# shenwei356/wfa

Measured on AMD Instinct MI355X. Metric: aligned pairs/sec (and Gcells/s) on 1e6 synthetic 1 kbp pairs @5% error, higher is better.
Workload: dtype u32; 1 GPU; 1000000 x 1000 bp pairs/GPU @5% error, global gap-affine 4/6/2, wf-adaptive 10/50/1, seed 3; config=c3, pairs_per_gpu=1000000, length=1000, parallelism=pair-sharded x1, ranks_seen_by_collective=1, backend=none (1 GPU), collective_forced=False, status_ok=1000000, setup_steps=0, gather=none (1 GPU), gather_bytes_per_rank_step=0, packed_pairs=1000000, retried_pairs=831

## Files before the change

wfa_amd/csrc/wfa_duo.hpp:

```cpp
#pragma once
#include "wfa_blk.hpp"
#include "wfa_duo_cfg.hpp"
#include "wfa_pk16.hpp"

namespace wfa {

struct DuoRed {
#define WFA_DUO_3(opa, opb, opc)                                                                                    \
    unsigned long long sv;                                                                                          \
    asm volatile("s_nop 1\n\t" opa " %0, %0, %0 " WFA_DPP_CTL_XOR1 "\n\t" opb " %1, %1, %1 " WFA_DPP_CTL_XOR1 "\n\t" opc \
        " %2, %2, %2 " WFA_DPP_CTL_XOR1 "\n\t" opa " %0, %0, %0 " WFA_DPP_CTL_XOR2 "\n\t" opb " %1, %1, %1 "        \
        WFA_DPP_CTL_XOR2 "\n\t" opc " %2, %2, %2 " WFA_DPP_CTL_XOR2 "\n\t" opa " %0, %0, %0 " WFA_DPP_CTL_HMIR "\n\t" \
        opb " %1, %1, %1 " WFA_DPP_CTL_HMIR "\n\t" opc " %2, %2, %2 " WFA_DPP_CTL_HMIR "\n\t"                         \
        "s_and_saveexec_b64 %3, %4\n\t" opa " %0, %0, %0 " WFA_DPP_CTL_MIR "\n\t" opb " %1, %1, %1 " WFA_DPP_CTL_MIR    \
        "\n\t" opc " %2, %2, %2 " WFA_DPP_CTL_MIR "\n\ts_mov_b64 exec, %3"                                            \
        : "+v"(a), "+v"(b), "+v"(c), "=&s"(sv)                                                                      \
        : "s"(wm)                                                                                                   \
        : "scc");
#define WFA_DUO_2(opa, opb)                                                                                         \
    unsigned long long sv;                                                                                          \
    asm volatile("s_nop 1\n\t" opa " %0, %0, %0 " WFA_DPP_CTL_XOR1 "\n\t" opb " %1, %1, %1 " WFA_DPP_CTL_XOR1 "\n\ts_nop 0\n\t" \
        opa " %0, %0, %0 " WFA_DPP_CTL_XOR2 "\n\t" opb " %1, %1, %1 " WFA_DPP_CTL_XOR2 "\n\ts_nop 0\n\t" opa        \
        " %0, %0, %0 " WFA_DPP_CTL_HMIR "\n\t" opb " %1, %1, %1 " WFA_DPP_CTL_HMIR "\n\t"                            \
        "s_and_saveexec_b64 %2, %3\n\t" opa " %0, %0, %0 " WFA_DPP_CTL_MIR "\n\t" opb " %1, %1, %1 " WFA_DPP_CTL_MIR    \
// ... 37 lines not shown

    const uint32_t  SW = P.lds_seq_words, PW = P.prepack_words;
    const uint32_t  FP = duo_fetch_pairs(PW), NBUF = duo_bufs(PW);
    uint32_t *const park0 = lds + NBUF * PW;
    const uint64_t  cap      = P.arena_words;
    const int       mdd      = (int)P.max_dist_diff;
    const int       minwf    = (int)P.min_wf_len;
    const bool      adaptive = P.adaptive != 0;
    const uint32_t  seed_si  = P.dx;
    uint32_t        pk_one   = 0x00010001u;
    if constexpr (PK) asm volatile("" : "+s"(pk_one));
    const int       rows_cap = (int)(cap / 32);

    int       st = 0;
    bool      wide = false;
    uint32_t  pidx = 0, si = 0, cells = 0, sbuf = 0;
    int       n = 0, m = 0, kb = 0;
    bool      slow = false, first_eq = false;
    int             j = l7, k0 = 0;
    uint32_t        mdn = 0u, mup = 0u;
    const uint32_t *lq = lds + 4, *lt = lds + 4;
    uint32_t       *rowp = nullptr;

    uint32_t M[R][RW], I[RW], D[RW];
    int      rlo[R], rhi[R];
    int      lim[PP], lmx[PP];
#pragma unroll
    for (int d = 0; d < R; d++) {
        rlo[d] = BK_BIG, rhi[d] = -BK_BIG;
#pragma unroll
        for (int p = 0; p < RW; p++) M[d][p] = 0u;
    }
#pragma unroll
    for (int p = 0; p < RW; p++) I[p] = D[p] = 0u;
#pragma unroll
    for (int p = 0; p < PP; p++) lim[p] = 0, lmx[p] = 0;

    uint32_t buf_free  = (1u << NBUF) - 1u;
    uint32_t park_used = 0u;
    constexpr uint32_t PF_TOK = 1u, PF_LD = 2u, PF_STAGED = 4u, PF_DRY = 8u;
    uint32_t pf = 0u;
    uint32_t pf_tok = 0u, pf_ld_idx = 0u, pf_idx = 0u, pf_buf = 0u;
    uint32_t st_mask = 0u;
    uint4    pf_w = make_uint4(0u, 0u, 0u, 0u);

#ifdef WFA_STAMPS
    unsigned long long stamp_acc[8] = {0, 0, 0, 0, 0, 0, 0, 0}, stamp_prev;
    unsigned long long evt[8] = {0, 0, 0, 0, 0, 0, 0, 0};
    asm volatile("s_memtime %0\n\ts_waitcnt lgkmcnt(0)" : "=s"(stamp_prev)::"memory");
#endif
    const auto pair_of = [&](uint32_t idx) { return P.work ? P.work[idx] : P.chunk_first + idx; };
    const auto dn1 = [&](uint32_t x) { return (uint32_t)__builtin_amdgcn_update_dpp(0, (int)x, 0x111, 0xf, 0xf, true) & mdn; };
    const auto up1 = [&](uint32_t x) { return (uint32_t)__builtin_amdgcn_update_dpp(0, (int)x, 0x101, 0xf, 0xf, true) & mup; };
    const auto other_half = [&](int x) { return __builtin_amdgcn_update_dpp(0, x, 0x128, 0xf, 0xf, true); };
    const auto set_derived = [&]() {
        j   = wide ? l15 : l7;
        mdn = j == 0 ? 0u : ~0u;
        mup = j == (wide ? 15 : 7) ? 0u : ~0u;
        k0  = kb + PP * j;
#pragma unroll
        for (int p = 0; p < PP; p++) lim[p] = imax2(1, imin2(n + k0 + p, m)), lmx[p] = imax2(n + k0 + p, m);
        lq   = lds + sbuf * PW + 4u;
        lt   = lq + SW;
        if constexpr (DUO_ARENA_FMT == 10u)
            rowp = P.arena + (uint64_t)pidx * cap + (((uint32_t)k0 & 56u) >> 3) * (uint32_t)(rows_cap * 4) + (((uint32_t)k0 >> 2) & 1u) * 16u;
        else if constexpr (DUO_ARENA_FMT == 9u)
            rowp = P.arena + (uint64_t)pidx * cap + (((uint32_t)k0 & 60u) >> 2) * (uint32_t)(rows_cap * 2) + si * 2u;
        else
            rowp = P.arena + (uint64_t)pidx * cap + (uint64_t)(si >> 3) * 256u + (si & 7u) * 2u;
    };
    const auto clear_rings = [&]() {
#pragma unroll
        for (int d = 0; d < R; d++) {
            rlo[d] = BK_BIG, rhi[d] = -BK_BIG;
#pragma unroll
            for (int p = 0; p < RW; p++) M[d][p] = 0u;
        }
#pragma unroll
        for (int p = 0; p < RW; p++) I[p] = D[p] = 0u;
    };
    const auto or_halves = [&](uint32_t v) {
        uint32_t r = 0u;
#pragma unroll
        for (int o = 0; o < 8; o++) r |= (uint32_t)__builtin_amdgcn_readlane((int)v, 8 * o);
        return r;
    };

    const auto refill = [&](auto ph_c) __attribute__((always_inline)) -> bool {
        constexpr int ph  = decltype(ph_c)::value;
        constexpr int NEW = (ph + R - 1) % R;
        pf        = (uint32_t)__builtin_amdgcn_readfirstlane((int)pf);
        park_used = (uint32_t)__builtin_amdgcn_readfirstlane((int)park_used);
        buf_free  = (uint32_t)__builtin_amdgcn_readfirstlane((int)buf_free);
        st_mask   = (uint32_t)__builtin_amdgcn_readfirstlane((int)st_mask);
        if ((pf & (PF_LD | PF_STAGED)) == PF_LD) {
            const uint32_t cnt = umin2(FP, P.chunk_n - pf_ld_idx);
            st_mask = 0u;
            {
                uint32_t f = buf_free;
                for (uint32_t c = 0; c < cnt; c++) st_mask |= f & (0u - f), f &= f - 1u;
            }
            buf_free &= ~st_mask;
            const uint32_t w0 = (uint32_t)lane * 4u, slot = w0 / PW;
            if (slot < cnt) {
                uint32_t f = st_mask;
                for (uint32_t c = 0; c < slot; c++) f &= f - 1u;
                const uint32_t b = (uint32_t)__builtin_ctz(f);
                *reinterpret_cast<uint4 *>(lds + b * PW + (w0 - slot * PW)) = pf_w;
            }
            pf_idx = pf_ld_idx, pf = (pf | PF_STAGED) & ~PF_LD;
        }
        if ((pf & (PF_TOK | PF_LD)) == PF_TOK) {
            pf_ld_idx = (uint32_t)__builtin_amdgcn_readfirstlane((int)pf_tok);
            const bool have = pf_ld_idx < P.chunk_n;
            if (have) {
                const uint32_t *const slot = P.prepack + (uint64_t)pf_ld_idx * PW;
                const uint32_t cnt = umin2(FP, P.chunk_n - pf_ld_idx);
                if ((uint32_t)lane * 4u < cnt * PW) pf_w = *reinterpret_cast<const uint4 *>(slot + lane * 4);
            }
            pf = (pf & ~PF_TOK) | (have ? PF_LD : PF_DRY);
        }
        if ((pf & (PF_TOK | PF_DRY)) == 0u) {
            if (lane == 0) pf_tok = atomicAdd(P.queue_head, FP);
            pf |= PF_TOK;
        }
        unsigned long long m_free;
        WFA_STAMP(0);
        for (;;) {
        const bool run   = st == 1;
        const int  Wc    = wide ? 64 : 32;
        const bool touch = run && rhi[NEW] >= rlo[NEW] && (rlo[NEW] <= kb || rhi[NEW] >= kb + Wc - 1);
        bool       narrowable = false;
        if constexpr (ph == 0) {
            int ulo = rlo[0], uhi = rhi[0];
#pragma unroll
            for (int d = 1; d < R; d++) ulo = imin2(ulo, rlo[d]), uhi = imax2(uhi, rhi[d]);
            narrowable    = run && wide && uhi - ulo + 1 <= DUO_NARROW_AT;
        }
        const unsigned long long m_ev = __ballot(touch || narrowable);
        m_free = __ballot(st == 0);
        if (__builtin_expect(!(m_ev != 0ull || (m_free != 0ull && (park_used != 0u || (pf & PF_STAGED) != 0u))), 1)) break;
        WFA_EVT(1, 1);
        {
            int ulo = rlo[0], uhi = rhi[0];
#pragma unroll
            for (int d = 1; d < R; d++) ulo = imin2(ulo, rlo[d]), uhi = imax2(uhi, rhi[d]);
            const int span = uhi - ulo + 1;
            int act = 0;
            if (touch) act = wide ? (span > DUO_WIDE_MAX ? 4 : 1) : (span > DUO_WIDEN_AT ? 2 : 1);
            else if (narrowable) act = 3;
            const int Wn  = act == 2 ? 64 : (act == 3 ? 32 : Wc);
            const int kbn = (((ulo + uhi + 1 - Wn) >> 1) + 2) & ~3;
            if (act != 0 && act != 4 && !(ulo - kbn >= 1 && uhi - kbn <= Wn - 2)) act = 4;
            const int  o_act = other_half(act), o_kb = other_half(kb), o_kbn = other_half(kbn);
            const bool o_wide = other_half(wide ? 1 : 0) != 0;
            bool widen  = act == 2 && !(hi_half && o_act == 2);
            bool taken  = !wide && !o_wide && o_act == 2 && !(!hi_half && act == 2);
            bool evict  = taken && st == 1;
            unsigned long long m_evict = __ballot(evict);
            bool               lost    = false;
            while (m_evict != 0ull) {
                const int      l0   = __builtin_ctzll(m_evict);
                const uint32_t oct  = (uint32_t)l0 >> 3;
                m_evict &= ~(0xFFull << (8 * oct));
                const bool mine = evict && ((uint32_t)lane >> 3) == oct;
                if (park_used == (1u << DUO_PARK) - 1u) {
                    if (((uint32_t)lane >> 3) == (oct ^ 1u)) lost = true;
                    if (mine) evict = false, taken = false;
                    continue;
                }
                const uint32_t rec = (uint32_t)__builtin_ctz(~park_used);
                park_used |= 1u << rec;
                WFA_EVT(3, 1);
                uint32_t *const pr = park0 + rec * DUO_PARK_WORDS;
                if (mine) {
                    uint4 *const w = reinterpret_cast<uint4 *>(pr + 12 * l7);
                    const auto pk  = [](uint32_t lo, uint32_t hi) { return lo | (hi << 16); };
                    const auto pk2 = [&](const uint32_t(&v)[RW], int h) -> uint32_t {
                        if constexpr (PK) return v[h];
                        else return pk(v[2 * h], v[2 * h + 1]);
                    };
                    uint32_t pw[8];
                    int      plo[4], phi[4];
#pragma unroll
                    for (int r = 0; r < 4; r++) {
                        pw[2 * r]     = r < R ? pk2(M[(ph + r) % R], 0) : 0u;
                        pw[2 * r + 1] = r < R ? pk2(M[(ph + r) % R], 1) : 0u;
                        plo[r] = r < R ? rlo[(ph + r) % R] : BK_BIG, phi[r] = r < R ? rhi[(ph + r) % R] : -BK_BIG;
                    }
                    w[0] = make_uint4(pw[0], pw[1], pw[2], pw[3]);
                    if constexpr (R > 2) w[1] = make_uint4(pw[4], pw[5], pw[6], pw[7]);
                    w[2] = make_uint4(pk2(I, 0), pk2(I, 1), pk2(D, 0), pk2(D, 1));
                    if (l7 == 0) {
                        uint4 *const s4 = reinterpret_cast<uint4 *>(pr + 96);
                        s4[0] = make_uint4(pidx, si, cells, sbuf);
                        s4[1] = make_uint4((uint32_t)n, (uint32_t)m, (uint32_t)kb, (slow ? 1u : 0u) | (first_eq ? 2u : 0u));
                        s4[2] = make_uint4((uint32_t)plo[0], (uint32_t)plo[1], (uint32_t)plo[2], (uint32_t)plo[3]);
                        s4[3] = make_uint4((uint32_t)phi[0], (uint32_t)phi[1], (uint32_t)phi[2], (uint32_t)phi[3]);
                    }
                }
            }
            if (lost) widen = false, act = 4;
            {
                const bool o_lost = other_half(lost ? 1 : 0) != 0;
                if (o_lost) taken = false;
            }
            if (__ballot(act == 4) != 0ull) {
                WFA_EVT(7, __builtin_popcountll(__ballot(act == 4 && j == 0)));
                if (act == 4 && j == 0) {
                    P.pair_meta[pidx] = make_uint4(ST_REDO_BAND, 0u, 0u, 0u);
                    push_redo(P, pair_of(pidx), ST_REDO_BAND);
                }
                buf_free |= or_halves(act == 4 ? (1u << sbuf) : 0u);
                if (act == 4) {
                    st = 0, wide = false;
                    clear_rings();
                }
            }
            const int  rb   = lane & ~15;
            const bool join = taken;
            int src = lane;
            bool moved = false, freed = false;
            {
                if (join) {
                    const int Bo = (lane & ~7) ^ 8, dl = (o_kbn - o_kb) >> 2, jo = (lane - rb) + dl;
                    src = (jo >= 0 && jo < 8) ? Bo + jo : -1, moved = true;
                } else if (act == 1) {
                    const int Bo = wide ? rb : (lane & ~7), Go = wide ? 16 : 8, dl = (kbn - kb) >> 2, jo = (lane - Bo) + dl;
// ... 13 lines not shown
                const int sl = (src < 0 ? lane : src) << 2;
#pragma unroll
                for (int d = 0; d < R; d++)
#pragma unroll
                    for (int p = 0; p < RW; p++) {
                        const uint32_t v = (uint32_t)__builtin_amdgcn_ds_bpermute(sl, (int)M[d][p]);
                        M[d][p]          = src < 0 ? 0u : v;
                    }
#pragma unroll
                for (int p = 0; p < RW; p++) {
                    const uint32_t v = (uint32_t)__builtin_amdgcn_ds_bpermute(sl, (int)I[p]);
                    const uint32_t u = (uint32_t)__builtin_amdgcn_ds_bpermute(sl, (int)D[p]);
                    I[p] = src < 0 ? 0u : v, D[p] = src < 0 ? 0u : u;
                }
                if (__ballot(join) != 0ull) {
                    const int      o_n = other_half(n), o_m = other_half(m);
                    const uint32_t o_pidx = (uint32_t)other_half((int)pidx), o_si = (uint32_t)other_half((int)si);
                    const uint32_t o_cells = (uint32_t)other_half((int)cells), o_sbuf = (uint32_t)other_half((int)sbuf);
                    const int      o_fl = other_half((slow ? 1 : 0) | (first_eq ? 2 : 0));
                    int o_rlo[R], o_rhi[R];
#pragma unroll
                    for (int d = 0; d < R; d++) o_rlo[d] = other_half(rlo[d]), o_rhi[d] = other_half(rhi[d]);
                    if (join) {
                        n = o_n, m = o_m, pidx = o_pidx, si = o_si, cells = o_cells, sbuf = o_sbuf;
                        slow = (o_fl & 1) != 0, first_eq = (o_fl & 2) != 0;
#pragma unroll
                        for (int d = 0; d < R; d++) rlo[d] = o_rlo[d], rhi[d] = o_rhi[d];
                        st = 1;
                    }
                }
                if (join) kb = o_kbn;
                else if (moved && !freed) kb = kbn;
                if (join || widen) wide = true;
                if (act == 3) wide = false;
                if (freed) {
                    st = 0;
#pragma unroll
                    for (int d = 0; d < R; d++) rlo[d] = BK_BIG, rhi[d] = -BK_BIG;
                }
            }
            m_free = __ballot(st == 0);
            while (m_free != 0ull && (park_used != 0u || (pf & PF_STAGED) != 0u)) {
                const uint32_t oct  = (uint32_t)__builtin_ctzll(m_free) >> 3;
                const bool     mine = ((uint32_t)lane >> 3) == oct;
                if (park_used != 0u) {
                    const uint32_t rec = (uint32_t)__builtin_ctz(park_used);
                    park_used &= park_used - 1u;
                    WFA_EVT(4, 1);
                    const uint32_t *const pr = park0 + rec * DUO_PARK_WORDS;
                    if (mine) {
                        const uint4 *const w = reinterpret_cast<const uint4 *>(pr + 12 * l7);
                        const uint4 v0 = w[0], v1 = R > 2 ? w[1] : make_uint4(0u, 0u, 0u, 0u), v2 = w[2];
                        const uint32_t pw[8] = {v0.x, v0.y, v0.z, v0.w, v1.x, v1.y, v1.z, v1.w};
                        const uint4 *const s4 = reinterpret_cast<const uint4 *>(pr + 96);
                        const uint4 a0 = s4[0], a1 = s4[1], a2 = s4[2], a3 = s4[3];
                        const uint32_t plo[4] = {a2.x, a2.y, a2.z, a2.w}, phi[4] = {a3.x, a3.y, a3.z, a3.w};
#pragma unroll
                        for (int r = 0; r < R; r++) {
                            if constexpr (PK) {
                                M[(ph + r) % R][0] = pw[2 * r], M[(ph + r) % R][1] = pw[2 * r + 1];
                            } else {
                                M[(ph + r) % R][0] = pw[2 * r] & 0xFFFFu, M[(ph + r) % R][1] = pw[2 * r] >> 16;
                                M[(ph + r) % R][2] = pw[2 * r + 1] & 0xFFFFu, M[(ph + r) % R][3] = pw[2 * r + 1] >> 16;
                            }
                            rlo[(ph + r) % R] = (int)plo[r], rhi[(ph + r) % R] = (int)phi[r];
                        }
                        if constexpr (PK) {
                            I[0] = v2.x, I[1] = v2.y, D[0] = v2.z, D[1] = v2.w;
                        } else {
                            I[0] = v2.x & 0xFFFFu, I[1] = v2.x >> 16, I[2] = v2.y & 0xFFFFu, I[3] = v2.y >> 16;
                            D[0] = v2.z & 0xFFFFu, D[1] = v2.z >> 16, D[2] = v2.w & 0xFFFFu, D[3] = v2.w >> 16;
                        }
                        pidx = a0.x, si = a0.y, cells = a0.z, sbuf = a0.w;
                        n = (int)a1.x, m = (int)a1.y, kb = (int)a1.z, slow = (a1.w & 1u) != 0u, first_eq = (a1.w & 2u) != 0u;
                        st = 1, wide = false;
                    }
                    m_free &= ~(0xFFull << (8 * oct));
                    continue;
                }
                pf_buf   = (uint32_t)__builtin_ctz(st_mask);
                st_mask &= st_mask - 1u;
                const uint32_t this_idx = pf_idx;
                pf_idx += 1u;
                const uint32_t *const hb = lds + pf_buf * PW;
                const uint32_t nq = (uint32_t)__builtin_amdgcn_readfirstlane((int)hb[0]), mt = (uint32_t)__builtin_amdgcn_readfirstlane((int)hb[1]);
                const uint32_t status = (uint32_t)__builtin_amdgcn_readfirstlane((int)hb[2]);
                if (st_mask == 0u) pf &= ~PF_STAGED;
                if (status != ST_PENDING) {
                    if (lane == 0) {
                        P.pair_meta[this_idx] = make_uint4(status, 0u, 0u, 0u);
                        if (status >= ST_REDO_BYTES) push_redo(P, pair_of(this_idx), status);
                    }
                    buf_free |= 1u << pf_buf;
                    continue;
                }
                WFA_EVT(5, 1);
                if (mine) {
                    pidx = this_idx, sbuf = pf_buf;
                    n = (int)nq, m = (int)mt;
                    const int Ak = m - n;
                    si = 0, cells = 0, slow = false;
                    kb = -16 + PP * imax2(-3, imin2(3, Ak / (2 * PP)));
                    first_eq = ((hb[4] ^ hb[4 + SW]) & 3u) == 0u;
                    clear_rings();
                    st = 1, wide = false;
                }
                m_free &= ~(0xFFull << (8 * oct));
            }
            set_derived();
            __builtin_amdgcn_fence(__ATOMIC_RELEASE, "wavefront");
            __builtin_amdgcn_fence(__ATOMIC_ACQUIRE, "wavefront");
        }
        }
        WFA_STAMP(1);
        return m_free == ~0ull && park_used == 0u && (pf & (PF_DRY | PF_LD | PF_STAGED)) == PF_DRY;
    };

    const auto step = [&](auto ph_c) __attribute__((always_inline)) {
        constexpr int ph = decltype(ph_c)::value;
        const bool run = (st == 1);
        const unsigned long long wm = __ballot(wide);
        WFA_EVT(0, 1), WFA_EVT(6, __builtin_popcountll(__ballot(run)) / 8);

        uint32_t(&Mo)[RW] = M[(ph + R - DOE) % R];
        uint32_t(&Mx)[RW] = M[(ph + R - DX) % R];
        uint32_t(&Mn)[RW] = M[ph];

        uint32_t nM[PP], nI[RW], nD[RW], wd[RW], cc[PP];
        const uint32_t a_edge = dn1(Mo[RW - 1]), b_edge = dn1(I[RW - 1]);
        const uint32_t c_edge = up1(Mo[0]), d_edge = up1(D[0]);
        const bool     slow_any = __ballot(run && slow) != 0ull;
        const auto next_slow = [&](const uint32_t(&Mo4)[PP], const uint32_t(&I4)[PP], const uint32_t(&D4)[PP], const uint32_t(&Mx4)[PP],
                                   uint32_t ae, uint32_t be, uint32_t ce, uint32_t de, uint32_t(&nI4)[PP], uint32_t(&nD4)[PP],
                                   uint32_t(&wd4)[PP]) __attribute__((always_inline)) {
#pragma unroll
            for (int p = 0; p < PP; p++) {
                const int      k  = k0 + p;
                const uint32_t a0 = p ? Mo4[p - 1] : ae, b0 = p ? I4[p - 1] : be;
                const uint32_t c0 = p < PP - 1 ? Mo4[p + 1] : ce, d0 = p < PP - 1 ? D4[p + 1] : de;
                const uint32_t x0 = Mx4[p];
                const uint32_t a = (int)a0 > m ? 0u : a0, b = (int)b0 > m ? 0u : b0;
                const uint32_t c = (int)c0 - k > n ? 0u : c0, d = (int)d0 - k > n ? 0u : d0;
                const uint32_t x = ((int)x0 > m || (int)x0 - k > n) ? 0u : x0;
                const uint32_t mi = umax2(a, b), tI = umin2(mi, 1u), Isk = mi + tI;
                const uint32_t Dsk = umax2(c, d), tD = umin2(Dsk, 1u);
                const uint32_t x1  = x + umin2(x, 1u);
                const uint32_t Msk = umax3(Isk, Dsk, x1);
                const bool fromX = x != 0u && Msk == x1;
                const bool fromI = !fromX && Msk == Isk;
                const uint32_t mu = umax2(a0, b0), Iu = mu + umin2(mu, 1u), Du = umax2(c0, d0);
                const uint32_t Xu = x0 + umin2(x0, 1u);
                const bool     iext = a < b, dext = c < d;
                const uint32_t o0   = (fromI && iext) ? Iu : ((!fromX && !fromI && dext) ? Du : umax3(Iu, Du, Xu));
                const bool     kin  = k >= -(n - 1) && k <= m - 1;
                nM[p] = kin ? Msk : 0u, nI4[p] = kin ? Isk : 0u, nD4[p] = kin ? Dsk : 0u;
                wd4[p] = blk_word(o0, iext, dext, fromX, fromI);
                cc[p]  = (CENSUS && kin) ? tI + tD + umin2(Msk, 1u) : 0u;
            }
        };
        if constexpr (PK) {
            if (__builtin_expect(!slow_any, 1)) {
                const uint32_t a0 = __builtin_amdgcn_alignbit(Mo[0], a_edge, 16), a1 = __builtin_amdgcn_alignbit(Mo[1], Mo[0], 16);
                const uint32_t c1 = __builtin_amdgcn_alignbit(c_edge, Mo[1], 16);
                const uint32_t b0 = __builtin_amdgcn_alignbit(I[0], b_edge, 16), b1 = __builtin_amdgcn_alignbit(I[1], I[0], 16);
                const uint32_t d0 = __builtin_amdgcn_alignbit(D[1], D[0], 16), d1 = __builtin_amdgcn_alignbit(d_edge, D[1], 16);
                uint32_t M2[2];
                wide_next2<true>(wide_pk(a0), wide_pk(b0), wide_pk(a1) , wide_pk(d0), wide_pk(Mx[0]), wide_pk(pk_one),
                                  M2[0], nI[0], nD[0], wd[0]);
                wide_next2<true>(wide_pk(a1), wide_pk(b1), wide_pk(c1), wide_pk(d1), wide_pk(Mx[1]), wide_pk(pk_one), M2[1], nI[1], nD[1], wd[1]);
#pragma unroll
                for (int p = 0; p < PP; p++) {
                    const int sh = 16 * (p & 1);
                    nM[p] = (M2[p >> 1] >> sh) & 0xFFFFu;
                    cc[p] = CENSUS ? (((nI[p >> 1] >> sh) & 0xFFFFu) != 0u ? 1u : 0u) + (((nD[p >> 1] >> sh) & 0xFFFFu) != 0u ? 1u : 0u) +
                                         (nM[p] != 0u ? 1u : 0u)
                                   : 0u;
                }
            } else {
                uint32_t Mo4[PP], I4[PP], D4[PP], Mx4[PP], nI4[PP], nD4[PP], wd4[PP];
#pragma unroll
                for (int p = 0; p < PP; p++) {
                    const int sh = 16 * (p & 1);
                    Mo4[p] = (Mo[p >> 1] >> sh) & 0xFFFFu, I4[p] = (I[p >> 1] >> sh) & 0xFFFFu;
                    D4[p] = (D[p >> 1] >> sh) & 0xFFFFu, Mx4[p] = (Mx[p >> 1] >> sh) & 0xFFFFu;
                }
                next_slow(Mo4, I4, D4, Mx4, a_edge >> 16, b_edge >> 16, c_edge & 0xFFFFu, d_edge & 0xFFFFu, nI4, nD4, wd4);
#pragma unroll
                for (int h = 0; h < 2; h++)
                    nI[h] = nI4[2 * h] | (nI4[2 * h + 1] << 16), nD[h] = nD4[2 * h] | (nD4[2 * h + 1] << 16),
                    wd[h] = wd4[2 * h] | (wd4[2 * h + 1] << 16);
            }
        } else if (__builtin_expect(!slow_any, 1)) {
#pragma unroll
            for (int p = 0; p < PP; p++) {
                const uint32_t a = p ? Mo[p - 1] : a_edge, b = p ? I[p - 1] : b_edge;
                const uint32_t c = p < PP - 1 ? Mo[p + 1] : c_edge, d = p < PP - 1 ? D[p + 1] : d_edge;
                const uint32_t x = Mx[p];
                const uint32_t mi = umax2(a, b), Isk = mi + (mi != 0u ? 1u : 0u);
                const uint32_t Dsk = umax2(c, d);
                const uint32_t x1  = x + (x != 0u ? 1u : 0u);
                const uint32_t Msk = umax3(Isk, Dsk, x1);
                nM[p] = Msk, nI[p] = Isk, nD[p] = Dsk;
                wd[p] = blk_word_asm(Msk, a, b, c, d, x1, umax2(Isk, Dsk), Isk, Dsk);
                cc[p] = CENSUS ? (mi != 0u ? 1u : 0u) + (Dsk != 0u ? 1u : 0u) + (Msk != 0u ? 1u : 0u) : 0u;
            }
        } else {
            next_slow(Mo, I, D, Mx, a_edge, b_edge, c_edge, d_edge, nI, nD, wd);
        }
        if (__builtin_expect(__ballot(run && si <= seed_si) != 0ull, 0)) {
            const bool want = run && ((si == 0u && first_eq) || (si == seed_si && !first_eq));
#pragma unroll
            for (int p = 0; p < PP; p++)
                if (want && k0 + p == 0 && nM[p] == 0u) {
                    const uint32_t sw = first_eq ? BLK_SEED_MATCH : BLK_SEED_MISMATCH;
                    nM[p] = 1u, cc[p] = CENSUS ? 1u : 0u;
                    if constexpr (PK) wd[p >> 1] = (p & 1) ? (wd[p >> 1] & 0xFFFFu) | (sw << 16) : (wd[p >> 1] & 0xFFFF0000u) | sw;
                    else wd[p] = sw;
                }
        }
        const bool no_room = run && (int)si >= rows_cap;
        {
            uint32_t anyc = 0u;
// ... 37 lines not shown
            } while (__ballot(go) != 0ull);
#pragma unroll
            for (int p = 0; p < PP; p++)
                if (psel == p) nM[p] = (uint32_t)h;
            cmask &= cmask - 1u;
        }
        WFA_STAMP(3);

        bool nz[PP], hit[PP], hitl = false;
#pragma unroll
        for (int p = 0; p < PP; p++) nz[p] = nM[p] != 0u, hit[p] = nM[p] >= (uint32_t)lim[p], hitl |= hit[p];
        bool       term    = false;
        const bool hit_any = __ballot(hitl) != 0ull;
        bool       ghit    = false;
        if (hit_any) {
            bool tl = false;
#pragma unroll
            for (int p = 0; p < PP; p++) tl |= (k0 + p == m - n && nz[p] && (int)nM[p] >= m);
            const int r = DuoRed::or1((hitl ? 1 : 0) | (tl ? 2 : 0), wm);
            ghit = (r & 1) != 0;
            slow |= ghit;
            term = run && (r & 2) != 0;
        }

        int      ilo = 0, ihi = -1;
        bool     anyM = false;
        uint32_t csum = 0u;
        if (__builtin_expect(!hit_any, 1)) {
            constexpr int ABSENT = BK_BIG + 1;
            int glo = BK_BIG, ghi = -BK_BIG, dd[PP];
#pragma unroll
// ... 85 lines not shown
        }
        if constexpr (DUO_ARENA_FMT != 10u) rowp += 2;
        if constexpr (DUO_ARENA_FMT == 7u) rowp += (((uint32_t)(uintptr_t)rowp & 0x38u) == 0u) ? 240 : 0;

        if constexpr (PK) {
#pragma unroll
            for (int h = 0; h < 2; h++) {
                Mn[h] = nM[2 * h] | (nM[2 * h + 1] << 16);
                I[h]  = wide_u32(__builtin_elementwise_min(wide_pk(nI[h]), wide_pk(Mn[h])));
                D[h]  = wide_u32(__builtin_elementwise_min(wide_pk(nD[h]), wide_pk(Mn[h])));
            }
        } else {
#pragma unroll
            for (int p = 0; p < PP; p++) Mn[p] = nM[p], I[p] = nI[p], D[p] = nD[p];
        }
        rlo[ph] = keepl ? kb + ilo : BK_BIG;
        rhi[ph] = keepl ? kb + ihi : -BK_BIG;

        const bool fin = run && (term || no_room);
        if (__ballot(fin) != 0ull) {
            const int ctot = (CENSUS && P.census) ? (int)cells : 0;
            int hf   = 0;
#pragma unroll
            for (int p = 0; p < PP; p++)
                if (k0 + p == m - n) hf = (int)nM[p];
            hf = DuoRed::max1(hf, wm);
            if (fin && j == 0) {
                if (no_room) {
                    P.pair_meta[pidx] = make_uint4(ST_REDO_ARENA, 0u, 0u, 0u);
                    push_redo(P, pair_of(pidx), ST_REDO_ARENA);
                } else {
                    P.pair_meta[pidx] = make_uint4(ST_OK, si * P.g, (uint32_t)hf, (uint32_t)ctot);
                }
            }
            buf_free |= or_halves(fin ? (1u << sbuf) : 0u);
            if (fin) {
                st = 0, wide = false;
                clear_rings();
            }
        }
        if (run && !fin) si += 1u;
        WFA_STAMP(5);
    };

    for (;;) {
        if (refill(std::integral_constant<int, 0>{})) break;
        step(std::integral_constant<int, 0>{});
        if constexpr (R > 1) {
            if (refill(std::integral_constant<int, 1 % R>{})) break;
            step(std::integral_constant<int, 1 % R>{});
// ... 5 lines not shown
        if constexpr (R > 3) {
            if (refill(std::integral_constant<int, 3 % R>{})) break;
            step(std::integral_constant<int, 3 % R>{});
        }
    }
#ifdef WFA_STAMPS
    if (lane == 0 && P.debug_info) {
        unsigned long long *acc = reinterpret_cast<unsigned long long *>(P.debug_info);
        for (int i = 0; i < 8; i++) atomicAdd(acc + i, stamp_acc[i]);
        for (int i = 0; i < 8; i++) atomicAdd(acc + 8 + i, evt[i]);
    }
#endif
}

#ifndef WFA_DUO_VGPRS
#define WFA_DUO_VGPRS 64
#endif
static_assert(16u * (256u - 4u) / 2u < 2048u, "wfa_duo_kernel's packed rings need offsets under 4 096");
template <bool CENSUS, int DX = 2, int DOE = 4>
__global__ __launch_bounds__(64, WFA_DUO_WAVES) __attribute__((amdgpu_num_vgpr(WFA_DUO_VGPRS))) void wfa_duo_kernel(const KParams P) {
    duo_run<CENSUS, DX, DOE, true>(P);
}
template <bool CENSUS, int DX = 2, int DOE = 4>
__global__ __launch_bounds__(64, WFA_DUO_WAVES) __attribute__((amdgpu_num_vgpr(WFA_DUO_VGPRS))) void wfa_duo32_kernel(const KParams P) {
    duo_run<CENSUS, DX, DOE, false>(P);
}

}
```

wfa_amd/csrc/wfa_duo_cfg.hpp:

```cpp
#pragma once
#include "wfa_common.hpp"

namespace wfa {

#ifndef WFA_DUO_WAVES
#define WFA_DUO_WAVES 4
#endif
#ifndef WFA_DUO_PARK
#define WFA_DUO_PARK 4
#endif
#ifndef WFA_DUO_WIDEN_AT
#define WFA_DUO_WIDEN_AT 26
#endif
#ifndef WFA_DUO_NARROW_AT
#define WFA_DUO_NARROW_AT 21
#endif
#ifndef WFA_DUO_GROUP_MAJOR
#define WFA_DUO_GROUP_MAJOR 2
#endif
constexpr uint32_t DUO_ARENA_FMT = WFA_DUO_GROUP_MAJOR == 2 ? 10u : WFA_DUO_GROUP_MAJOR == 1 ? 9u : 7u;
constexpr int DUO_PARK       = WFA_DUO_PARK;
constexpr int DUO_PARK_WORDS = 8 * 12 + 16;
constexpr int DUO_BUFS       = 8 + 1 + DUO_PARK;
constexpr int DUO_FETCH_MAX  = 8;
constexpr int DUO_WIDEN_AT   = WFA_DUO_WIDEN_AT;
constexpr int DUO_NARROW_AT  = WFA_DUO_NARROW_AT;
constexpr int DUO_WIDE_MAX   = 56;

__host__ __device__ inline uint32_t duo_fetch_pairs(uint32_t prepack_words) {
    const uint32_t f = 256u / prepack_words;
    return f < 1u ? 1u : (f > (uint32_t)DUO_FETCH_MAX ? (uint32_t)DUO_FETCH_MAX : f);
}
__host__ __device__ inline uint32_t duo_bufs(uint32_t prepack_words) { return 8u + duo_fetch_pairs(prepack_words) + (uint32_t)DUO_PARK; }
__host__ __device__ inline uint32_t duo_lds_words(uint32_t prepack_words) {
    return duo_bufs(prepack_words) * prepack_words + (uint32_t)DUO_PARK * DUO_PARK_WORDS;
}

hipError_t wfa_launch_duo(int shape, const KParams &P, uint32_t grid, size_t lds_bytes, hipStream_t st, bool census, bool pk);

}
```

Before: 62.64 million pairs/s.

## Cut VGPR pressure to fit five waves: move per-pair state to LDS headers

Per-pair scalars (n, m, pidx, sbuf) are no longer held in registers. They are read from a header in each pair's LDS sequence buffer. Ring bounds are packed as two 16-bit halves in one register, edge masks become booleans, and the slow-path cell update is inlined per cell. Parked pairs release their sequence buffer and are later re-fetched from global prepack memory, which removes the park buffers from LDS. The VGPR budget drops to 48 so WFA_DUO_WAVES can rise to 5, trading extra LDS reads and global refetches for higher occupancy.

```diff
diff --git a/wfa_amd/csrc/wfa_duo.hpp b/wfa_amd/csrc/wfa_duo.hpp
--- a/wfa_amd/csrc/wfa_duo.hpp
+++ b/wfa_amd/csrc/wfa_duo.hpp
@@ -75,20 +75,23 @@
 
     int       st = 0;
     bool      wide = false;
-    uint32_t  pidx = 0, si = 0, cells = 0, sbuf = 0;
-    int       n = 0, m = 0, kb = 0;
+    uint32_t  si = 0, cells = 0;
+    int       kb = 0;
     bool      slow = false, first_eq = false;
     int             j = l7, k0 = 0;
-    uint32_t        mdn = 0u, mup = 0u;
-    const uint32_t *lq = lds + 4, *lt = lds + 4;
+    bool            gfirst = true, glast = true;
+    uint32_t *lq = lds + 4, *lt = lds + 4;
     uint32_t       *rowp = nullptr;
 
     uint32_t M[R][RW], I[RW], D[RW];
-    int      rlo[R], rhi[R];
+    typedef short rb_pair __attribute__((ext_vector_type(2)));
+    constexpr int      RB_BIG   = 0x7000;
+    constexpr uint32_t RB_EMPTY = (uint32_t)RB_BIG | ((uint32_t)(-RB_BIG) << 16);
+    uint32_t rbnd[R];
     int      lim[PP], lmx[PP];
 #pragma unroll
     for (int d = 0; d < R; d++) {
-        rlo[d] = BK_BIG, rhi[d] = -BK_BIG;
+        rbnd[d] = RB_EMPTY;
 #pragma unroll
         for (int p = 0; p < RW; p++) M[d][p] = 0u;
     }
@@ -96,10 +99,22 @@
     for (int p = 0; p < RW; p++) I[p] = D[p] = 0u;
 #pragma unroll
     for (int p = 0; p < PP; p++) lim[p] = 0, lmx[p] = 0;
+    const auto rb_lo = [&](int d) { return (int)(short)(rbnd[d] & 0xFFFFu); };
+    const auto rb_hi = [&](int d) { return (int)rbnd[d] >> 16; };
+    const auto rb_union = [&](int &ulo, int &uhi) {
+        rb_pair lo = __builtin_bit_cast(rb_pair, rbnd[0]), hi = lo;
+#pragma unroll
+        for (int d = 1; d < R; d++) {
+            const rb_pair v = __builtin_bit_cast(rb_pair, rbnd[d]);
+            lo = __builtin_elementwise_min(lo, v), hi = __builtin_elementwise_max(hi, v);
+        }
+        ulo = (int)lo.x, uhi = (int)hi.y;
+    };
 
     uint32_t buf_free  = (1u << NBUF) - 1u;
     uint32_t park_used = 0u;
     constexpr uint32_t PF_TOK = 1u, PF_LD = 2u, PF_STAGED = 4u, PF_DRY = 8u;
+    constexpr uint32_t PF_LDRES = 16u, PF_STRES = 32u, PF_LDREC = 0xF00u, PF_STREC = 0xF000u;
     uint32_t pf = 0u;
     uint32_t pf_tok = 0u, pf_ld_idx = 0u, pf_idx = 0u, pf_buf = 0u;
     uint32_t st_mask = 0u;
@@ -111,17 +126,31 @@
     asm volatile("s_memtime %0\n\ts_waitcnt lgkmcnt(0)" : "=s"(stamp_prev)::"memory");
 #endif
     const auto pair_of = [&](uint32_t idx) { return P.work ? P.work[idx] : P.chunk_first + idx; };
-    const auto dn1 = [&](uint32_t x) { return (uint32_t)__builtin_amdgcn_update_dpp(0, (int)x, 0x111, 0xf, 0xf, true) & mdn; };
-    const auto up1 = [&](uint32_t x) { return (uint32_t)__builtin_amdgcn_update_dpp(0, (int)x, 0x101, 0xf, 0xf, true) & mup; };
+    const auto dn1 = [&](uint32_t x) {
+        const uint32_t v = (uint32_t)__builtin_amdgcn_update_dpp(0, (int)x, 0x111, 0xf, 0xf, true);
+        return gfirst ? 0u : v;
+    };
+    const auto up1 = [&](uint32_t x) {
+        const uint32_t v = (uint32_t)__builtin_amdgcn_update_dpp(0, (int)x, 0x101, 0xf, 0xf, true);
+        return glast ? 0u : v;
+    };
     const auto other_half = [&](int x) { return __builtin_amdgcn_update_dpp(0, x, 0x128, 0xf, 0xf, true); };
+    const auto hdr_n = [&]() { return (int)lq[-4]; };
+    const auto hdr_m = [&]() { return (int)lq[-3]; };
+    const auto hdr_sbuf = [&]() { return lq[-2]; };
+    const auto hdr_pidx = [&]() { return lq[-1]; };
+    const auto set_limits = [&](int n, int m) {
+#pragma unroll
+        for (int p = 0; p < PP; p++) lim[p] = imax2(1, imin2(n + k0 + p, m)), lmx[p] = imax2(n + k0 + p, m);
+    };
     const auto set_derived = [&]() {
+        const int      n = hdr_n(), m = hdr_m();
+        const uint32_t pidx = hdr_pidx();
         j   = wide ? l15 : l7;
-        mdn = j == 0 ? 0u : ~0u;
-        mup = j == (wide ? 15 : 7) ? 0u : ~0u;
+        gfirst = j == 0;
+        glast  = j == (wide ? 15 : 7);
         k0  = kb + PP * j;
-#pragma unroll
-        for (int p = 0; p < PP; p++) lim[p] = imax2(1, imin2(n + k0 + p, m)), lmx[p] = imax2(n + k0 + p, m);
-        lq   = lds + sbuf * PW + 4u;
+        set_limits(n, m);
         lt   = lq + SW;
         if constexpr (DUO_ARENA_FMT == 10u)
             rowp = P.arena + (uint64_t)pidx * cap + (((uint32_t)k0 & 56u) >> 3) * (uint32_t)(rows_cap * 4) + (((uint32_t)k0 >> 2) & 1u) * 16u;
@@ -133,7 +162,7 @@
     const auto clear_rings = [&]() {
 #pragma unroll
         for (int d = 0; d < R; d++) {
-            rlo[d] = BK_BIG, rhi[d] = -BK_BIG;
+            rbnd[d] = RB_EMPTY;
 #pragma unroll
             for (int p = 0; p < RW; p++) M[d][p] = 0u;
         }
@@ -155,7 +184,8 @@
         buf_free  = (uint32_t)__builtin_amdgcn_readfirstlane((int)buf_free);
         st_mask   = (uint32_t)__builtin_amdgcn_readfirstlane((int)st_mask);
         if ((pf & (PF_LD | PF_STAGED)) == PF_LD) {
-            const uint32_t cnt = umin2(FP, P.chunk_n - pf_ld_idx);
+            const bool     res = (pf & PF_LDRES) != 0u;
+            const uint32_t cnt = res ? 1u : umin2(FP, P.chunk_n - pf_ld_idx);
             st_mask = 0u;
             {
                 uint32_t f = buf_free;
@@ -169,7 +199,15 @@
                 const uint32_t b = (uint32_t)__builtin_ctz(f);
                 *reinterpret_cast<uint4 *>(lds + b * PW + (w0 - slot * PW)) = pf_w;
             }
-            pf_idx = pf_ld_idx, pf = (pf | PF_STAGED) & ~PF_LD;
+            if (!res) pf_idx = pf_ld_idx;
+            pf = ((pf | PF_STAGED) & ~(PF_LD | PF_LDRES | PF_STRES | PF_STREC)) | (res ? PF_STRES | ((pf & PF_LDREC) << 4) : 0u);
+        }
+        const uint32_t park_wait = park_used & ~((pf & PF_STRES) != 0u ? 1u << ((pf & PF_STREC) >> 12) : 0u);
+        if ((pf & PF_LD) == 0u && park_wait != 0u) {
+            const uint32_t rec  = (uint32_t)__builtin_ctz(park_wait);
+            const uint32_t ridx = (uint32_t)__builtin_amdgcn_readfirstlane((int)park0[rec * DUO_PARK_WORDS + 96u]);
+            if ((uint32_t)lane * 4u < PW) pf_w = *reinterpret_cast<const uint4 *>(P.prepack + (uint64_t)ridx * PW + lane * 4);
+            pf = (pf & ~PF_LDREC) | PF_LD | PF_LDRES | (rec << 8);
         }
         if ((pf & (PF_TOK | PF_LD)) == PF_TOK) {
             pf_ld_idx = (uint32_t)__builtin_amdgcn_readfirstlane((int)pf_tok);
@@ -190,22 +228,21 @@
         for (;;) {
         const bool run   = st == 1;
         const int  Wc    = wide ? 64 : 32;
-        const bool touch = run && rhi[NEW] >= rlo[NEW] && (rlo[NEW] <= kb || rhi[NEW] >= kb + Wc - 1);
+        const int  nlo = rb_lo(NEW), nhi = rb_hi(NEW);
+        const bool touch = run && nhi >= nlo && (nlo <= kb || nhi >= kb + Wc - 1);
         bool       narrowable = false;
         if constexpr (ph == 0) {
-            int ulo = rlo[0], uhi = rhi[0];
-#pragma unroll
-            for (int d = 1; d < R; d++) ulo = imin2(ulo, rlo[d]), uhi = imax2(uhi, rhi[d]);
+            int ulo, uhi;
+            rb_union(ulo, uhi);
             narrowable    = run && wide && uhi - ulo + 1 <= DUO_NARROW_AT;
         }
         const unsigned long long m_ev = __ballot(touch || narrowable);
         m_free = __ballot(st == 0);
-        if (__builtin_expect(!(m_ev != 0ull || (m_free != 0ull && (park_used != 0u || (pf & PF_STAGED) != 0u))), 1)) break;
+        if (__builtin_expect(!(m_ev != 0ull || (m_free != 0ull && (pf & PF_STAGED) != 0u)), 1)) break;
         WFA_EVT(1, 1);
         {
-            int ulo = rlo[0], uhi = rhi[0];
-#pragma unroll
-            for (int d = 1; d < R; d++) ulo = imin2(ulo, rlo[d]), uhi = imax2(uhi, rhi[d]);
+            int ulo, uhi;
+            rb_union(ulo, uhi);
             const int span = uhi - ulo + 1;
             int act = 0;
             if (touch) act = wide ? (span > DUO_WIDE_MAX ? 4 : 1) : (span > DUO_WIDEN_AT ? 2 : 1);
@@ -219,6 +256,7 @@
             bool taken  = !wide && !o_wide && o_act == 2 && !(!hi_half && act == 2);
             bool evict  = taken && st == 1;
             unsigned long long m_evict = __ballot(evict);
+            const uint32_t     my_sbuf = hdr_sbuf();
             bool               lost    = false;
             while (m_evict != 0ull) {
                 const int      l0   = __builtin_ctzll(m_evict);
@@ -232,6 +270,7 @@
                 }
                 const uint32_t rec = (uint32_t)__builtin_ctz(~park_used);
                 park_used |= 1u << rec;
+                buf_free |= 1u << (uint32_t)__builtin_amdgcn_readlane((int)my_sbuf, l0);
                 WFA_EVT(3, 1);
                 uint32_t *const pr = park0 + rec * DUO_PARK_WORDS;
                 if (mine) {
@@ -242,22 +281,21 @@
                         else return pk(v[2 * h], v[2 * h + 1]);
                     };
                     uint32_t pw[8];
-                    int      plo[4], phi[4];
+                    uint32_t prb[4];
 #pragma unroll
                     for (int r = 0; r < 4; r++) {
                         pw[2 * r]     = r < R ? pk2(M[(ph + r) % R], 0) : 0u;
                         pw[2 * r + 1] = r < R ? pk2(M[(ph + r) % R], 1) : 0u;
-                        plo[r] = r < R ? rlo[(ph + r) % R] : BK_BIG, phi[r] = r < R ? rhi[(ph + r) % R] : -BK_BIG;
+                        prb[r] = r < R ? rbnd[(ph + r) % R] : RB_EMPTY;
                     }
                     w[0] = make_uint4(pw[0], pw[1], pw[2], pw[3]);
                     if constexpr (R > 2) w[1] = make_uint4(pw[4], pw[5], pw[6], pw[7]);
                     w[2] = make_uint4(pk2(I, 0), pk2(I, 1), pk2(D, 0), pk2(D, 1));
                     if (l7 == 0) {
                         uint4 *const s4 = reinterpret_cast<uint4 *>(pr + 96);
-                        s4[0] = make_uint4(pidx, si, cells, sbuf);
-                        s4[1] = make_uint4((uint32_t)n, (uint32_t)m, (uint32_t)kb, (slow ? 1u : 0u) | (first_eq ? 2u : 0u));
-                        s4[2] = make_uint4((uint32_t)plo[0], (uint32_t)plo[1], (uint32_t)plo[2], (uint32_t)plo[3]);
-                        s4[3] = make_uint4((uint32_t)phi[0], (uint32_t)phi[1], (uint32_t)phi[2], (uint32_t)phi[3]);
+                        s4[0] = make_uint4(hdr_pidx(), si, CENSUS ? cells : 0u, 0u);
+                        s4[1] = make_uint4(0u, 0u, (uint32_t)kb, (slow ? 1u : 0u) | (first_eq ? 2u : 0u));
+                        s4[2] = make_uint4(prb[0], prb[1], prb[2], prb[3]);
                     }
                 }
             }
@@ -269,10 +307,11 @@
             if (__ballot(act == 4) != 0ull) {
                 WFA_EVT(7, __builtin_popcountll(__ballot(act == 4 && j == 0)));
                 if (act == 4 && j == 0) {
+                    const uint32_t pidx = hdr_pidx();
                     P.pair_meta[pidx] = make_uint4(ST_REDO_BAND, 0u, 0u, 0u);
                     push_redo(P, pair_of(pidx), ST_REDO_BAND);
                 }
-                buf_free |= or_halves(act == 4 ? (1u << sbuf) : 0u);
+                buf_free |= or_halves(act == 4 ? (1u << my_sbuf) : 0u);
                 if (act == 4) {
                     st = 0, wide = false;
                     clear_rings();
@@ -316,18 +355,18 @@
                     I[p] = src < 0 ? 0u : v, D[p] = src < 0 ? 0u : u;
                 }
                 if (__ballot(join) != 0ull) {
-                    const int      o_n = other_half(n), o_m = other_half(m);
-                    const uint32_t o_pidx = (uint32_t)other_half((int)pidx), o_si = (uint32_t)other_half((int)si);
-                    const uint32_t o_cells = (uint32_t)other_half((int)cells), o_sbuf = (uint32_t)other_half((int)sbuf);
+                    const uint32_t o_si = (uint32_t)other_half((int)si);
+                    const uint32_t o_cells = CENSUS ? (uint32_t)other_half((int)cells) : 0u;
+                    const int      o_lq = other_half((int)(lq - lds));
                     const int      o_fl = other_half((slow ? 1 : 0) | (first_eq ? 2 : 0));
-                    int o_rlo[R], o_rhi[R];
-#pragma unroll
-                    for (int d = 0; d < R; d++) o_rlo[d] = other_half(rlo[d]), o_rhi[d] = other_half(rhi[d]);
+                    uint32_t o_rb[R];
+#pragma unroll
+                    for (int d = 0; d < R; d++) o_rb[d] = (uint32_t)other_half((int)rbnd[d]);
                     if (join) {
-                        n = o_n, m = o_m, pidx = o_pidx, si = o_si, cells = o_cells, sbuf = o_sbuf;
+                        si = o_si, cells = o_cells, lq = lds + o_lq;
                         slow = (o_fl & 1) != 0, first_eq = (o_fl & 2) != 0;
 #pragma unroll
-                        for (int d = 0; d < R; d++) rlo[d] = o_rlo[d], rhi[d] = o_rhi[d];
+                        for (int d = 0; d < R; d++) rbnd[d] = o_rb[d];
                         st = 1;
                     }
                 }
@@ -338,16 +377,19 @@
                 if (freed) {
                     st = 0;
 #pragma unroll
-                    for (int d = 0; d < R; d++) rlo[d] = BK_BIG, rhi[d] = -BK_BIG;
+                    for (int d = 0; d < R; d++) rbnd[d] = RB_EMPTY;
                 }
             }
             m_free = __ballot(st == 0);
-            while (m_free != 0ull && (park_used != 0u || (pf & PF_STAGED) != 0u)) {
+            while (m_free != 0ull && (pf & PF_STAGED) != 0u) {
                 const uint32_t oct  = (uint32_t)__builtin_ctzll(m_free) >> 3;
                 const bool     mine = ((uint32_t)lane >> 3) == oct;
-                if (park_used != 0u) {
-                    const uint32_t rec = (uint32_t)__builtin_ctz(park_used);
-                    park_used &= park_used - 1u;
+                pf_buf   = (uint32_t)__builtin_ctz(st_mask);
+                st_mask &= st_mask - 1u;
+                if ((pf & PF_STRES) != 0u) {
+                    const uint32_t rec = (pf & PF_STREC) >> 12;
+                    park_used &= ~(1u << rec);
+                    pf &= ~(PF_STAGED | PF_STRES | PF_STREC);
                     WFA_EVT(4, 1);
                     const uint32_t *const pr = park0 + rec * DUO_PARK_WORDS;
                     if (mine) {
@@ -355,8 +397,8 @@
                         const uint4 v0 = w[0], v1 = R > 2 ? w[1] : make_uint4(0u, 0u, 0u, 0u), v2 = w[2];
                         const uint32_t pw[8] = {v0.x, v0.y, v0.z, v0.w, v1.x, v1.y, v1.z, v1.w};
                         const uint4 *const s4 = reinterpret_cast<const uint4 *>(pr + 96);
-                        const uint4 a0 = s4[0], a1 = s4[1], a2 = s4[2], a3 = s4[3];
-                        const uint32_t plo[4] = {a2.x, a2.y, a2.z, a2.w}, phi[4] = {a3.x, a3.y, a3.z, a3.w};
+                        const uint4 a0 = s4[0], a1 = s4[1], a2 = s4[2];
+                        const uint32_t prb[4] = {a2.x, a2.y, a2.z, a2.w};
 #pragma unroll
                         for (int r = 0; r < R; r++) {
                             if constexpr (PK) {
@@ -365,7 +407,7 @@
                                 M[(ph + r) % R][0] = pw[2 * r] & 0xFFFFu, M[(ph + r) % R][1] = pw[2 * r] >> 16;
                                 M[(ph + r) % R][2] = pw[2 * r + 1] & 0xFFFFu, M[(ph + r) % R][3] = pw[2 * r + 1] >> 16;
                             }
-                            rlo[(ph + r) % R] = (int)plo[r], rhi[(ph + r) % R] = (int)phi[r];
+                            rbnd[(ph + r) % R] = prb[r];
                         }
                         if constexpr (PK) {
                             I[0] = v2.x, I[1] = v2.y, D[0] = v2.z, D[1] = v2.w;
@@ -373,15 +415,15 @@
                             I[0] = v2.x & 0xFFFFu, I[1] = v2.x >> 16, I[2] = v2.y & 0xFFFFu, I[3] = v2.y >> 16;
                             D[0] = v2.z & 0xFFFFu, D[1] = v2.z >> 16, D[2] = v2.w & 0xFFFFu, D[3] = v2.w >> 16;
                         }
-                        pidx = a0.x, si = a0.y, cells = a0.z, sbuf = a0.w;
-                        n = (int)a1.x, m = (int)a1.y, kb = (int)a1.z, slow = (a1.w & 1u) != 0u, first_eq = (a1.w & 2u) != 0u;
+                        si = a0.y, cells = CENSUS ? a0.z : 0u;
+                        lq = lds + pf_buf * PW + 4u;
+                        if (l7 == 0) lq[-2] = pf_buf, lq[-1] = a0.x;
+                        kb = (int)a1.z, slow = (a1.w & 1u) != 0u, first_eq = (a1.w & 2u) != 0u;
                         st = 1, wide = false;
                     }
                     m_free &= ~(0xFFull << (8 * oct));
                     continue;
                 }
-                pf_buf   = (uint32_t)__builtin_ctz(st_mask);
-                st_mask &= st_mask - 1u;
                 const uint32_t this_idx = pf_idx;
                 pf_idx += 1u;
                 const uint32_t *const hb = lds + pf_buf * PW;
@@ -398,9 +440,9 @@
                 }
                 WFA_EVT(5, 1);
                 if (mine) {
-                    pidx = this_idx, sbuf = pf_buf;
-                    n = (int)nq, m = (int)mt;
-                    const int Ak = m - n;
+                    lq = lds + pf_buf * PW + 4u;
+                    if (l7 == 0) lq[-2] = pf_buf, lq[-1] = this_idx;
+                    const int Ak = (int)mt - (int)nq;
                     si = 0, cells = 0, slow = false;
                     kb = -16 + PP * imax2(-3, imin2(3, Ak / (2 * PP)));
                     first_eq = ((hb[4] ^ hb[4 + SW]) & 3u) == 0u;
@@ -429,39 +471,33 @@
         uint32_t(&Mn)[RW] = M[ph];
 
         uint32_t nM[PP], nI[RW], nD[RW], wd[RW], cc[PP];
-        const uint32_t a_edge = dn1(Mo[RW - 1]), b_edge = dn1(I[RW - 1]);
-        const uint32_t c_edge = up1(Mo[0]), d_edge = up1(D[0]);
         const bool     slow_any = __ballot(run && slow) != 0ull;
-        const auto next_slow = [&](const uint32_t(&Mo4)[PP], const uint32_t(&I4)[PP], const uint32_t(&D4)[PP], const uint32_t(&Mx4)[PP],
-                                   uint32_t ae, uint32_t be, uint32_t ce, uint32_t de, uint32_t(&nI4)[PP], uint32_t(&nD4)[PP],
-                                   uint32_t(&wd4)[PP]) __attribute__((always_inline)) {
-#pragma unroll
-            for (int p = 0; p < PP; p++) {
-                const int      k  = k0 + p;
-                const uint32_t a0 = p ? Mo4[p - 1] : ae, b0 = p ? I4[p - 1] : be;
-                const uint32_t c0 = p < PP - 1 ? Mo4[p + 1] : ce, d0 = p < PP - 1 ? D4[p + 1] : de;
-                const uint32_t x0 = Mx4[p];
-                const uint32_t a = (int)a0 > m ? 0u : a0, b = (int)b0 > m ? 0u : b0;
-                const uint32_t c = (int)c0 - k > n ? 0u : c0, d = (int)d0 - k > n ? 0u : d0;
-                const uint32_t x = ((int)x0 > m || (int)x0 - k > n) ? 0u : x0;
-                const uint32_t mi = umax2(a, b), tI = umin2(mi, 1u), Isk = mi + tI;
-                const uint32_t Dsk = umax2(c, d), tD = umin2(Dsk, 1u);
-                const uint32_t x1  = x + umin2(x, 1u);
-                const uint32_t Msk = umax3(Isk, Dsk, x1);
-                const bool fromX = x != 0u && Msk == x1;
-                const bool fromI = !fromX && Msk == Isk;
-                const uint32_t mu = umax2(a0, b0), Iu = mu + umin2(mu, 1u), Du = umax2(c0, d0);
-                const uint32_t Xu = x0 + umin2(x0, 1u);
-                const bool     iext = a < b, dext = c < d;
-                const uint32_t o0   = (fromI && iext) ? Iu : ((!fromX && !fromI && dext) ? Du : umax3(Iu, Du, Xu));
-                const bool     kin  = k >= -(n - 1) && k <= m - 1;
-                nM[p] = kin ? Msk : 0u, nI4[p] = kin ? Isk : 0u, nD4[p] = kin ? Dsk : 0u;
-                wd4[p] = blk_word(o0, iext, dext, fromX, fromI);
-                cc[p]  = (CENSUS && kin) ? tI + tD + umin2(Msk, 1u) : 0u;
-            }
+        const auto slow_cell = [&](int p, int n, int m, uint32_t a0, uint32_t b0, uint32_t c0, uint32_t d0, uint32_t x0, uint32_t &nIp,
+                                   uint32_t &nDp, uint32_t &wdp) __attribute__((always_inline)) {
+            const int k = k0 + p;
+            const uint32_t a = (int)a0 > m ? 0u : a0, b = (int)b0 > m ? 0u : b0;
+            const uint32_t c = (int)c0 - k > n ? 0u : c0, d = (int)d0 - k > n ? 0u : d0;
+            const uint32_t x = ((int)x0 > m || (int)x0 - k > n) ? 0u : x0;
+            const uint32_t mi = umax2(a, b), tI = umin2(mi, 1u), Isk = mi + tI;
+            const uint32_t Dsk = umax2(c, d), tD = umin2(Dsk, 1u);
+            const uint32_t x1  = x + umin2(x, 1u);
+            const uint32_t Msk = umax3(Isk, Dsk, x1);
+            const bool fromX = x != 0u && Msk == x1;
+            const bool fromI = !fromX && Msk == Isk;
+            const uint32_t mu = umax2(a0, b0), Iu = mu + umin2(mu, 1u), Du = umax2(c0, d0);
+            const uint32_t Xu = x0 + umin2(x0, 1u);
+            const bool     iext = a < b, dext = c < d;
+            const uint32_t o0   = (fromI && iext) ? Iu : ((!fromX && !fromI && dext) ? Du : umax3(Iu, Du, Xu));
+            const bool     kin  = k >= -(n - 1) && k <= m - 1;
+            nM[p] = kin ? Msk : 0u, nIp = kin ? Isk : 0u, nDp = kin ? Dsk : 0u;
+            wdp   = blk_word(o0, iext, dext, fromX, fromI);
+            cc[p] = (CENSUS && kin) ? tI + tD + umin2(Msk, 1u) : 0u;
+            __builtin_amdgcn_sched_barrier(0);
         };
         if constexpr (PK) {
             if (__builtin_expect(!slow_any, 1)) {
+                const uint32_t a_edge = dn1(Mo[RW - 1]), b_edge = dn1(I[RW - 1]);
+                const uint32_t c_edge = up1(Mo[0]), d_edge = up1(D[0]);
                 const uint32_t a0 = __builtin_amdgcn_alignbit(Mo[0], a_edge, 16), a1 = __builtin_amdgcn_alignbit(Mo[1], Mo[0], 16);
                 const uint32_t c1 = __builtin_amdgcn_alignbit(c_edge, Mo[1], 16);
                 const uint32_t b0 = __builtin_amdgcn_alignbit(I[0], b_edge, 16), b1 = __builtin_amdgcn_alignbit(I[1], I[0], 16);
@@ -479,20 +515,22 @@
                                    : 0u;
                 }
             } else {
-                uint32_t Mo4[PP], I4[PP], D4[PP], Mx4[PP], nI4[PP], nD4[PP], wd4[PP];
+                const auto ex = [](const uint32_t(&V)[RW], int q) { return (V[q >> 1] >> (16 * (q & 1))) & 0xFFFFu; };
+                const int  n = hdr_n(), m = hdr_m();
+#pragma unroll
+                for (int h = 0; h < 2; h++) nI[h] = 0u, nD[h] = 0u, wd[h] = 0u;
 #pragma unroll
                 for (int p = 0; p < PP; p++) {
-                    const int sh = 16 * (p & 1);
-                    Mo4[p] = (Mo[p >> 1] >> sh) & 0xFFFFu, I4[p] = (I[p >> 1] >> sh) & 0xFFFFu;
-                    D4[p] = (D[p >> 1] >> sh) & 0xFFFFu, Mx4[p] = (Mx[p >> 1] >> sh) & 0xFFFFu;
-                }
-                next_slow(Mo4, I4, D4, Mx4, a_edge >> 16, b_edge >> 16, c_edge & 0xFFFFu, d_edge & 0xFFFFu, nI4, nD4, wd4);
-#pragma unroll
-                for (int h = 0; h < 2; h++)
-                    nI[h] = nI4[2 * h] | (nI4[2 * h + 1] << 16), nD[h] = nD4[2 * h] | (nD4[2 * h + 1] << 16),
-                    wd[h] = wd4[2 * h] | (wd4[2 * h + 1] << 16);
+                    uint32_t Ip, Dp, wp;
+                    slow_cell(p, n, m, p ? ex(Mo, p - 1) : dn1(Mo[RW - 1]) >> 16, p ? ex(I, p - 1) : dn1(I[RW - 1]) >> 16,
+                              p < PP - 1 ? ex(Mo, p + 1) : up1(Mo[0]) & 0xFFFFu, p < PP - 1 ? ex(D, p + 1) : up1(D[0]) & 0xFFFFu, ex(Mx, p), Ip, Dp, wp);
+                    nI[p >> 1] |= Ip << (16 * (p & 1)), nD[p >> 1] |= Dp << (16 * (p & 1)), wd[p >> 1] |= wp << (16 * (p & 1));
+                }
+                set_limits(n, m);
             }
         } else if (__builtin_expect(!slow_any, 1)) {
+            const uint32_t a_edge = dn1(Mo[RW - 1]), b_edge = dn1(I[RW - 1]);
+            const uint32_t c_edge = up1(Mo[0]), d_edge = up1(D[0]);
 #pragma unroll
             for (int p = 0; p < PP; p++) {
                 const uint32_t a = p ? Mo[p - 1] : a_edge, b = p ? I[p - 1] : b_edge;
@@ -507,7 +545,13 @@
                 cc[p] = CENSUS ? (mi != 0u ? 1u : 0u) + (Dsk != 0u ? 1u : 0u) + (Msk != 0u ? 1u : 0u) : 0u;
             }
         } else {
-            next_slow(Mo, I, D, Mx, a_edge, b_edge, c_edge, d_edge, nI, nD, wd);
+            const int n = hdr_n(), m = hdr_m();
+#pragma unroll
+            for (int p = 0; p < PP; p++)
+                slow_cell(p, n, m, p ? Mo[p - 1] : dn1(Mo[RW - 1]), p ? I[p - 1] : dn1(I[RW - 1]), p < PP - 1 ? Mo[p + 1] : up1(Mo[0]),
+                          p < PP - 1 ? D[p + 1] : up1(D[0]), Mx[p],
+                          nI[p], nD[p], wd[p]);
+            set_limits(n, m);
         }
         if (__builtin_expect(__ballot(run && si <= seed_si) != 0ull, 0)) {
             const bool want = run && ((si == 0u && first_eq) || (si == seed_si && !first_eq));
@@ -575,7 +619,8 @@
         const bool hit_any = __ballot(hitl) != 0ull;
         bool       ghit    = false;
         if (hit_any) {
-            bool tl = false;
+            bool      tl = false;
+            const int n = hdr_n(), m = hdr_m();
 #pragma unroll
             for (int p = 0; p < PP; p++) tl |= (k0 + p == m - n && nz[p] && (int)nM[p] >= m);
             const int r = DuoRed::or1((hitl ? 1 : 0) | (tl ? 2 : 0), wm);
@@ -691,26 +736,29 @@
 #pragma unroll
             for (int p = 0; p < PP; p++) Mn[p] = nM[p], I[p] = nI[p], D[p] = nD[p];
         }
-        rlo[ph] = keepl ? kb + ilo : BK_BIG;
-        rhi[ph] = keepl ? kb + ihi : -BK_BIG;
+        rbnd[ph] = keepl ? ((uint32_t)(kb + ilo) & 0xFFFFu) | ((uint32_t)(kb + ihi) << 16) : RB_EMPTY;
 
         const bool fin = run && (term || no_room);
         if (__ballot(fin) != 0ull) {
             const int ctot = (CENSUS && P.census) ? (int)cells : 0;
             int hf   = 0;
+            const int      Ak = hdr_m() - hdr_n();
+            const uint32_t pidx = hdr_pidx();
 #pragma unroll
             for (int p = 0; p < PP; p++)
-                if (k0 + p == m - n) hf = (int)nM[p];
+                if (k0 + p == Ak) hf = (int)nM[p];
             hf = DuoRed::max1(hf, wm);
             if (fin && j == 0) {
                 if (no_room) {
-                    P.pair_meta[pidx] = make_uint4(ST_REDO_ARENA, 0u, 0u, 0u);
-                    push_redo(P, pair_of(pidx), ST_REDO_ARENA);
+                    uint32_t z = 0u;
+                    asm volatile("" : "+v"(z));
+                    P.pair_meta[pidx] = make_uint4(ST_REDO_ARENA + z, z, z, z);
+                    push_redo(P, pair_of(pidx), ST_REDO_ARENA + z);
                 } else {
                     P.pair_meta[pidx] = make_uint4(ST_OK, si * P.g, (uint32_t)hf, (uint32_t)ctot);
                 }
             }
-            buf_free |= or_halves(fin ? (1u << sbuf) : 0u);
+            buf_free |= or_halves(fin ? (1u << hdr_sbuf()) : 0u);
             if (fin) {
                 st = 0, wide = false;
                 clear_rings();
@@ -746,7 +794,7 @@
 }
 
 #ifndef WFA_DUO_VGPRS
-#define WFA_DUO_VGPRS 64
+#define WFA_DUO_VGPRS 48
 #endif
 static_assert(16u * (256u - 4u) / 2u < 2048u, "wfa_duo_kernel's packed rings need offsets under 4 096");
 template <bool CENSUS, int DX = 2, int DOE = 4>
@@ -754,7 +802,7 @@
     duo_run<CENSUS, DX, DOE, true>(P);
 }
 template <bool CENSUS, int DX = 2, int DOE = 4>
-__global__ __launch_bounds__(64, WFA_DUO_WAVES) __attribute__((amdgpu_num_vgpr(WFA_DUO_VGPRS))) void wfa_duo32_kernel(const KParams P) {
+__global__ __launch_bounds__(64, 4) __attribute__((amdgpu_num_vgpr(64))) void wfa_duo32_kernel(const KParams P) {
     duo_run<CENSUS, DX, DOE, false>(P);
 }
 
diff --git a/wfa_amd/csrc/wfa_duo_cfg.hpp b/wfa_amd/csrc/wfa_duo_cfg.hpp
--- a/wfa_amd/csrc/wfa_duo_cfg.hpp
+++ b/wfa_amd/csrc/wfa_duo_cfg.hpp
@@ -4,7 +4,7 @@
 namespace wfa {
 
 #ifndef WFA_DUO_WAVES
-#define WFA_DUO_WAVES 4
+#define WFA_DUO_WAVES 5
 #endif
 #ifndef WFA_DUO_PARK
 #define WFA_DUO_PARK 4
@@ -21,7 +21,6 @@
 constexpr uint32_t DUO_ARENA_FMT = WFA_DUO_GROUP_MAJOR == 2 ? 10u : WFA_DUO_GROUP_MAJOR == 1 ? 9u : 7u;
 constexpr int DUO_PARK       = WFA_DUO_PARK;
 constexpr int DUO_PARK_WORDS = 8 * 12 + 16;
-constexpr int DUO_BUFS       = 8 + 1 + DUO_PARK;
 constexpr int DUO_FETCH_MAX  = 8;
 constexpr int DUO_WIDEN_AT   = WFA_DUO_WIDEN_AT;
 constexpr int DUO_NARROW_AT  = WFA_DUO_NARROW_AT;
@@ -31,7 +30,7 @@
     const uint32_t f = 256u / prepack_words;
     return f < 1u ? 1u : (f > (uint32_t)DUO_FETCH_MAX ? (uint32_t)DUO_FETCH_MAX : f);
 }
-__host__ __device__ inline uint32_t duo_bufs(uint32_t prepack_words) { return 8u + duo_fetch_pairs(prepack_words) + (uint32_t)DUO_PARK; }
+__host__ __device__ inline uint32_t duo_bufs(uint32_t prepack_words) { return 8u + duo_fetch_pairs(prepack_words); }
 __host__ __device__ inline uint32_t duo_lds_words(uint32_t prepack_words) {
     return duo_bufs(prepack_words) * prepack_words + (uint32_t)DUO_PARK * DUO_PARK_WORDS;
 }
```

After: 48.16 million pairs/s. -23.1%, worse.
